# ap229997/hands

Measured on AMD Instinct MI355X. Metric: hands/sec, higher is better.
Workload: dtype f32; 1 GPU; hands_light ResNet-50 x3 + feature_conv + HMR + MANO, 224x224, bz=256 samples/GPU (512 hands, 768 trunk passes); per_gpu_batch=256, global_batch=256, parallelism=dp1, rccl_ranks=1, launched_by=direct, conv3x3_stride1=winograd_f4x4:stages1234

## Files before the change

hands_amd/csrc/conv_igemm.hip:

```cpp
#include <hip/hip_runtime.h>
#include <stdint.h>
#include "hands_hip.h"
#include "common.h"

namespace {

typedef unsigned int u32x4 __attribute__((ext_vector_type(4)));
typedef double f64x4 __attribute__((ext_vector_type(4)));

__device__ __forceinline__ float gelu_erf(float x) { return x * 0.5f * (1.0f + erff(x * 0.70710678118654752440f)); }

__device__ __forceinline__ float4 apply_act(float4 v, int act) {
  if (act == HANDS_ACT_RELU) {
    v = relu_f32(v);
  } else if (act == HANDS_ACT_GELU) {
    v.x = gelu_erf(v.x); v.y = gelu_erf(v.y); v.z = gelu_erf(v.z); v.w = gelu_erf(v.w);
  } else if (act == HANDS_ACT_LEAKY_RELU) {
    v.x = v.x > 0.f ? v.x : 0.01f * v.x; v.y = v.y > 0.f ? v.y : 0.01f * v.y;
    v.z = v.z > 0.f ? v.z : 0.01f * v.z; v.w = v.w > 0.f ? v.w : 0.01f * v.w;
  }
  return v;
}

__device__ __forceinline__ float f4elem(const float4& v, int t) {
  return t == 0 ? v.x : (t == 1 ? v.y : (t == 2 ? v.z : v.w));
}

constexpr int BK = 16;
constexpr int LDS_ROW = 16;
constexpr int LDS_ROW_B3 = 24;

typedef __bf16 bf16x8 __attribute__((ext_vector_type(8)));

__device__ __forceinline__ void split3(float x, uint32_t& u0, uint32_t& u1, uint32_t& u2) {
  u0 = __float_as_uint(x) & 0xffff0000u;
  const float r1 = x - __uint_as_float(u0);
  u1 = __float_as_uint(r1) & 0xffff0000u;
  const float r2 = r1 - __uint_as_float(u1);
  u2 = __float_as_uint(r2);
}

__device__ __forceinline__ void store_split4(float* dst, float4 v) {
  uint32_t a0, a1, a2, b0, b1, b2, c0, c1, c2, d0, d1, d2;
  split3(v.x, a0, a1, a2); split3(v.y, b0, b1, b2); split3(v.z, c0, c1, c2); split3(v.w, d0, d1, d2);
  *reinterpret_cast<uint2*>(dst) = make_uint2((a0 >> 16) | b0, (c0 >> 16) | d0);
  *reinterpret_cast<uint2*>(dst + 8) = make_uint2((a1 >> 16) | b1, (c1 >> 16) | d1);
  *reinterpret_cast<uint2*>(dst + 16) = make_uint2((a2 >> 16) | (b2 & 0xffff0000u), (c2 >> 16) | (d2 & 0xffff0000u));
}

struct ConvArgs {
  const float* __restrict__ in;
  const float* __restrict__ w;
  const float* __restrict__ bias;
  const float* res;
  float* out;
  int M, N, Kpad;
  int H, W, Cin, Ho, Wo, KH, KW, stride, pad;
  int in_ps, out_ps, res_ps;
  int relu;
  int nblk_m, nblk_n;
  const float* __restrict__ in2;
  int K0, H2, W2, stride2, in2_ps;
  int ksplit;
  float* partial;
  int part_ps;
  const float* pre_scale;
  const float* pre_shift;
  int* counters = nullptr;
  const float* fin_res = nullptr;
  int fin_act = 0;
};

__device__ __forceinline__ int xcd_remap(int bid, int nwg) {
  const int q = nwg >> 3, r = nwg & 7;
  const int xcd = bid & 7, idx = bid >> 3;
  const int base = (xcd < r) ? xcd * (q + 1) : r * (q + 1) + (xcd - r) * q;
  return base + idx;
}

typedef float f32x2 __attribute__((ext_vector_type(2)));

constexpr int EROW = 68;
constexpr int EPI_FLOATS = 4 * 32 * EROW;
template <int ACT, bool RES>
__device__ __forceinline__ void epilogue_full(const f32x16 (&acc)[2][2], float* sE, int lane, const float* bias_p,
                                              const char* res_u, int res_ps, char* out_u, int out_ps) {
  const int half = lane >> 5;
  float* wr = sE + (lane & 31) * EROW + half * 4;
  const float* rd = sE + (lane >> 4) * EROW + (lane & 15) * 4;
  const uint32_t o_off = (uint32_t)((lane >> 4) * out_ps + (lane & 15) * 4) * 4u;
  const uint32_t r_off = (uint32_t)((lane >> 4) * res_ps + (lane & 15) * 4) * 4u;
  const float4 bv4 = *reinterpret_cast<const float4*>(bias_p);
#ifndef HANDS_EPI_SCALAR_ADDS
  const f32x2 b01 = {bv4.x, bv4.y}, b23 = {bv4.z, bv4.w};
#endif
#pragma unroll
  for (int j = 0; j < 2; ++j) {
#pragma unroll
    for (int i = 0; i < 2; ++i)
#pragma unroll
      for (int q = 0; q < 4; ++q)
        *reinterpret_cast<float4*>(wr + i * 32 + q * 8) =
            make_float4(acc[i][j][q * 4 + 0], acc[i][j][q * 4 + 1], acc[i][j][q * 4 + 2], acc[i][j][q * 4 + 3]);
    float4 rv[RES ? 8 : 1];
    if constexpr (RES) {
#pragma unroll
      for (int r = 0; r < 8; ++r)
        rv[r] = *reinterpret_cast<const float4*>(res_u + (size_t)(j * 32 + 4 * r) * (size_t)res_ps * 4 + r_off);
    }
#pragma unroll
    for (int r = 0; r < 8; ++r) {
      const float4 t = *reinterpret_cast<const float4*>(rd + 4 * r * EROW);
#ifdef HANDS_EPI_SCALAR_ADDS
      float4 v = make_float4(t.x + bv4.x, t.y + bv4.y, t.z + bv4.z, t.w + bv4.w);
      if constexpr (RES) { v.x += rv[r].x; v.y += rv[r].y; v.z += rv[r].z; v.w += rv[r].w; }
      asm volatile("" : "+v"(v.x), "+v"(v.y), "+v"(v.z), "+v"(v.w));
#else
      f32x2 v01 = {t.x, t.y}, v23 = {t.z, t.w};
      v01 = v01 + b01;
      v23 = v23 + b23;
      if constexpr (RES) {
        const f32x2 r01 = {rv[r].x, rv[r].y}, r23 = {rv[r].z, rv[r].w};
        v01 = v01 + r01;
        v23 = v23 + r23;
      }
      float4 v = make_float4(v01.x, v01.y, v23.x, v23.y);
#endif
      if constexpr (ACT != HANDS_ACT_NONE) v = apply_act(v, ACT);
      *reinterpret_cast<float4*>(out_u + (size_t)(j * 32 + 4 * r) * (size_t)out_ps * 4 + o_off) = v;
      if (r & 1) __builtin_amdgcn_sched_barrier(0);
    }
  }
}

template <int BM, int BN, bool F64>
__device__ __forceinline__ void splitk_fused_tail(const ConvArgs& a, float* lds, int tile, int m0, int n0, int wave_u) {
  const int tid = wave_u * 64 + (int)__builtin_amdgcn_mbcnt_hi(~0u, __builtin_amdgcn_mbcnt_lo(~0u, 0u));
  volatile int& s_last = *reinterpret_cast<volatile int*>(lds);
  asm volatile("s_waitcnt vmcnt(0)" ::: "memory");
  __syncthreads();
  if (tid == 0) {
    __builtin_amdgcn_fence(__ATOMIC_RELEASE, "agent");
    asm volatile("s_waitcnt vmcnt(0)" ::: "memory");
    const int old = __hip_atomic_fetch_add(a.counters + tile, 1, __ATOMIC_RELAXED, __HIP_MEMORY_SCOPE_AGENT);
    const int last = old == a.ksplit - 1;
    if (last) __hip_atomic_store(a.counters + tile, 0, __ATOMIC_RELAXED, __HIP_MEMORY_SCOPE_AGENT);
    s_last = last;
  }
  __syncthreads();
  if (!s_last) return;
  __builtin_amdgcn_fence(__ATOMIC_ACQUIRE, "agent");
  const size_t slice = (size_t)a.M * a.part_ps;
  if constexpr (F64) {
    const double* part = reinterpret_cast<const double*>(a.partial);
    for (int idx = tid; idx < BM * BN; idx += 256) {
      const int m = m0 + idx / BN, n = n0 + idx % BN;
      if (m >= a.M || n >= a.N) continue;
      const double* p = part + (size_t)m * a.part_ps + n;
      double v = p[0];
      for (int sl = 1; sl < a.ksplit; ++sl) v += p[sl * slice];
      float f = (float)(v + (double)a.bias[n]);
      if (a.fin_res) f += a.fin_res[(size_t)m * a.res_ps + n];
      if (a.fin_act == HANDS_ACT_RELU) f = relu_f32(f);
      else if (a.fin_act == HANDS_ACT_GELU) f = gelu_erf(f);
      else if (a.fin_act == HANDS_ACT_LEAKY_RELU) f = f > 0.f ? f : 0.01f * f;
      a.out[(size_t)m * a.out_ps + n] = f;
    }
  } else {
    constexpr int C4 = BN / 4;
    for (int idx = tid; idx < BM * C4; idx += 256) {
      const int m = m0 + idx / C4, n = n0 + (idx % C4) * 4;
      if (m >= a.M || n >= a.N) continue;
      const float* p = a.partial + (size_t)m * a.part_ps + n;
      float4 v = *reinterpret_cast<const float4*>(p);
      for (int sl = 1; sl < a.ksplit; ++sl) {
        const float4 q = *reinterpret_cast<const float4*>(p + sl * slice);
        v.x += q.x; v.y += q.y; v.z += q.z; v.w += q.w;
      }
      const float4 b = *reinterpret_cast<const float4*>(a.bias + n);
      v.x += b.x; v.y += b.y; v.z += b.z; v.w += b.w;
      if (a.fin_res) {
        const float4 r = *reinterpret_cast<const float4*>(a.fin_res + (size_t)m * a.res_ps + n);
        v.x += r.x; v.y += r.y; v.z += r.z; v.w += r.w;
      }
      *reinterpret_cast<float4*>(a.out + (size_t)m * a.out_ps + n) = apply_act(v, a.fin_act);
    }
  }
}

constexpr int SK_SLOT_FLOATS = 4 * 64 * 64;

__device__ __forceinline__ void tile_coords(const ConvArgs& a, int tile, int& mt, int& nt) {
  constexpr int RASTER_GM = 8;
  if (a.nblk_n >= 8 && a.nblk_m >= RASTER_GM) {
    const int per = RASTER_GM * a.nblk_n;
    const int gidx = tile / per, idx = tile - gidx * per;
    const int gm = min(RASTER_GM, a.nblk_m - gidx * RASTER_GM);
    nt = idx / gm; mt = gidx * RASTER_GM + (idx - nt * gm);
  } else { mt = tile / a.nblk_n; nt = tile - mt * a.nblk_n; }
}

template <int WAVES_M, int WAVES_N, int MODE, int PREC = 0, bool PRE = false, int BLK = 0>
__device__ __forceinline__ void conv_tile(const ConvArgs& a, float* lds, int tile, int split, int kt0, int kt1,
                                          const float* acc_in, float* acc_out) {
  constexpr int ROW = PREC == 1 ? LDS_ROW_B3 : LDS_ROW;
  constexpr bool F64 = PREC == 2;
  constexpr bool STEM = MODE == 1;
  constexpr bool DUAL = MODE == 2;
  constexpr int BM = 64 * WAVES_M;
  constexpr int BN = 64 * WAVES_N;
  constexpr int A_ROWS = BM / 64;
  constexpr int W_ROWS = BN / 64;
  static_assert(WAVES_M * WAVES_N == 4, "4 waves per block");

  float* sX = lds;
  float* sW = lds + 2 * BM * ROW;

  const int tid = threadIdx.x;
  const int lane = tid & 63;
  const int wave = tid >> 6;
  const int wm = wave / WAVES_N;
  const int wn = wave % WAVES_N;

  int mt, nt;
  tile_coords(a, tile, mt, nt);
  const int m0 = mt * BM, n0 = nt * BN;

  const int srow = tid >> 2;
  const int chunk = tid & 3;
  const int swz_chunk = chunk ^ ((srow >> 2) & 3);
  int x_base[A_ROWS];
  int x_hi0[A_ROWS], x_wi0[A_ROWS];
  bool x_ok[A_ROWS];
  int x_base2[DUAL ? A_ROWS : 1];
  uint32_t x_mask[MODE == 0 ? A_ROWS : 1];
  int x_offb[MODE == 0 ? A_ROWS : 1];
  int x_b[A_ROWS];
  const int HoWo = a.Ho * a.Wo;
  const bool same_pixel = DUAL && a.K0 >= a.Kpad && a.stride == 1 && a.H == a.Ho && a.W == a.Wo;
#pragma unroll
  for (int i = 0; i < A_ROWS; ++i) {
    const int m = m0 + srow + 64 * i;
    x_ok[i] = m < a.M;
    const int mm = x_ok[i] ? m : 0;
    if (same_pixel) {
      x_b[i] = 0; x_hi0[i] = 0; x_wi0[i] = 0;
      x_base[i] = mm * a.in_ps;
      if constexpr (DUAL) x_base2[i] = 0;
      continue;
    }
    const int b = mm / HoWo;
    const int rem = mm - b * HoWo;
    const int ho = rem / a.Wo;
    const int wo = rem - ho * a.Wo;
    x_b[i] = b;
    x_hi0[i] = ho * a.stride - a.pad;
    x_wi0[i] = wo * a.stride - a.pad;
    x_base[i] = ((b * a.H + x_hi0[i]) * a.W + x_wi0[i]) * a.in_ps;
    if constexpr (DUAL) {
      x_base2[i] = ((b * a.H2 + ho * a.stride2) * a.W2 + wo * a.stride2) * a.in2_ps;
    }
  }
  __amdgpu_buffer_rsrc_t x_rsrc = __builtin_amdgcn_make_buffer_rsrc(const_cast<float*>(a.in), 0, (int)0x80000000u, 0x00020000);
  if constexpr (MODE == 0) {
    const int b_w = __builtin_amdgcn_readfirstlane(x_b[0]);
    x_rsrc = __builtin_amdgcn_make_buffer_rsrc(const_cast<float*>(a.in) + (size_t)b_w * a.H * a.W * a.in_ps, 0,
                                               (int)0x80000000u, 0x00020000);
#pragma unroll
    for (int i = 0; i < A_ROWS; ++i) {
      const int hb = max(0, -x_hi0[i]), he = min(a.KH, a.H - x_hi0[i]);
      const int wb = max(0, -x_wi0[i]), we = min(a.KW, a.W - x_wi0[i]);
      const uint32_t hm = he > hb ? ((1u << he) - 1u) & ~((1u << hb) - 1u) : 0u;
      const uint32_t wm = we > wb ? ((1u << we) - 1u) & ~((1u << wb) - 1u) : 0u;
      x_mask[i] = (x_ok[i] && hm != 0u && wm != 0u) ? (hm | (wm << 16)) : 0u;
      x_offb[i] = (((((x_b[i] - b_w) * a.H + x_hi0[i]) * a.W + x_wi0[i]) * a.in_ps) + chunk * 4) * 4;
    }
  }
  int x_off1[DUAL ? A_ROWS : 1], x_off2[DUAL ? A_ROWS : 1];
  __amdgpu_buffer_rsrc_t x_rsrc2 = x_rsrc;
  if constexpr (DUAL) {
    const int base1 = __builtin_amdgcn_readfirstlane(x_base[0]);
    const int base2 = __builtin_amdgcn_readfirstlane(x_base2[0]);
    x_rsrc = __builtin_amdgcn_make_buffer_rsrc(const_cast<float*>(a.in) + base1, 0, (int)0x80000000u, 0x00020000);
    x_rsrc2 = __builtin_amdgcn_make_buffer_rsrc(const_cast<float*>(a.in2) + base2, 0, (int)0x80000000u, 0x00020000);
#pragma unroll
    for (int i = 0; i < A_ROWS; ++i) {
      x_off1[i] = x_ok[i] ? (x_base[i] - base1 + chunk * 4) * 4 : chunk * 16;
      x_off2[i] = x_ok[i] ? (x_base2[i] - base2 + chunk * 4) * 4 : chunk * 16;
    }
  }
  const __amdgpu_buffer_rsrc_t w_rsrc =
      __builtin_amdgcn_make_buffer_rsrc(const_cast<float*>(a.w) + (size_t)n0 * a.Kpad, 0, (int)0x80000000u, 0x00020000);
  int w_offb[W_ROWS];
#pragma unroll
  for (int i = 0; i < W_ROWS; ++i) w_offb[i] = ((srow + 64 * i) * a.Kpad + chunk * 4) * 4;

  float4 xr[A_ROWS], wr[W_ROWS];
  static_assert(!PRE || (MODE == 2 && PREC != 1), "the input affine + LeakyReLU exists for exact-fp32 pointwise layers");
  float4 psr = make_float4(1.f, 1.f, 1.f, 1.f), pbr = make_float4(0.f, 0.f, 0.f, 0.f);
  int kh = 0, kw = 0, c0 = 0, woff = 0;
  const int ntaps = a.KH * a.KW;
  const int cw = (a.Cin & 31) == 0 ? 2 * BK : BK;

#define LOAD_TILES(KT)                                                                              \
  do {                                                                                              \
    if constexpr (STEM) {                                                                           \
                                          \
      const int tap = (KT) * 4 + chunk;                                                             \
      const int tkh = tap / a.KW;                                                                   \
      const int tkw = tap - tkh * a.KW;                                                             \
      const int toff = (tkh * a.W + tkw) * a.in_ps;                                                 \
      _Pragma("unroll") for (int i = 0; i < A_ROWS; ++i) {                                          \
        const bool ok = x_ok[i] && tap < ntaps && (unsigned)(x_hi0[i] + tkh) < (unsigned)a.H &&     \
                        (unsigned)(x_wi0[i] + tkw) < (unsigned)a.W;                                 \
        xr[i] = ok ? *reinterpret_cast<const float4*>(a.in + (x_base[i] + toff))                    \
                   : make_float4(0.f, 0.f, 0.f, 0.f);                                               \
      }                                                                                             \
    } else if constexpr (DUAL) {                                                                    \
       \
       \
       \
      const bool second = (KT) * BK >= a.K0;                                                        \
      const int soff = ((KT) * BK - (second ? a.K0 : 0)) * 4;                                       \
      _Pragma("unroll") for (int i = 0; i < A_ROWS; ++i) {                                          \
        const u32x4 ld = second ? __builtin_amdgcn_raw_buffer_load_b128(x_rsrc2, x_off2[i], soff, 0) \
                                : __builtin_amdgcn_raw_buffer_load_b128(x_rsrc, x_off1[i], soff, 0);  \
        xr[i] = make_float4(__uint_as_float(ld.x), __uint_as_float(ld.y), __uint_as_float(ld.z), __uint_as_float(ld.w)); \
      }                                                                                             \
    } else {                                                                                        \
       \
       \
       \
      const bool kvalid = c0 < a.Cin;              \
      const uint32_t sel = kvalid ? ((1u << kh) | (0x10000u << kw)) : 0x80000000u;   \
      const int toffb = ((kh * a.W + kw) * a.in_ps + c0) * 4;                                       \
      _Pragma("unroll") for (int i = 0; i < A_ROWS; ++i) {                                          \
        const bool ok = (x_mask[i] & sel) == sel;                                                   \
        const u32x4 ld = __builtin_amdgcn_raw_buffer_load_b128(x_rsrc, ok ? x_offb[i] + toffb : (int)0x80000000u, 0, 0); \
        xr[i] = make_float4(__uint_as_float(ld.x), __uint_as_float(ld.y), __uint_as_float(ld.z), __uint_as_float(ld.w)); \
      }                                                                                             \
      woff = kvalid ? (kh * a.KW + kw) * a.Cin + c0 : (KT) * BK;                                    \
      c0 += BK;                                                                                     \
      if ((c0 & (cw - 1)) == 0) {              \
        c0 -= cw;                                                                                   \
        if (++kw == a.KW) { kw = 0; if (++kh == a.KH) { kh = 0; c0 += cw; } }                       \
      }                                                                                             \
    }                                                                                               \
    if constexpr (MODE != 0) woff = (KT) * BK;                                                      \
    if constexpr (PRE) {                                                                            \
      psr = *reinterpret_cast<const float4*>(a.pre_scale + (KT) * BK + chunk * 4);                  \
      pbr = *reinterpret_cast<const float4*>(a.pre_shift + (KT) * BK + chunk * 4);                  \
    }                                                                                               \
    _Pragma("unroll") for (int i = 0; i < W_ROWS; ++i) {                                            \
      const u32x4 ld = __builtin_amdgcn_raw_buffer_load_b128(w_rsrc, w_offb[i], woff * 4, 0);        \
      wr[i] = make_float4(__uint_as_float(ld.x), __uint_as_float(ld.y), __uint_as_float(ld.z), __uint_as_float(ld.w)); \
    }                                                                                               \
  } while (0)

#define STORE_TILES(BUF)                                                                            \
  do {                                                                                              \
    if constexpr (PRE) {                                                                            \
      _Pragma("unroll") for (int i = 0; i < A_ROWS; ++i) {                                          \
        float4 v = make_float4(xr[i].x * psr.x + pbr.x, xr[i].y * psr.y + pbr.y, xr[i].z * psr.z + pbr.z, xr[i].w * psr.w + pbr.w); \
        v.x = v.x > 0.f ? v.x : 0.01f * v.x; v.y = v.y > 0.f ? v.y : 0.01f * v.y;                   \
        v.z = v.z > 0.f ? v.z : 0.01f * v.z; v.w = v.w > 0.f ? v.w : 0.01f * v.w;                   \
        xr[i] = v;                                                                                  \
      }                                                                                             \
    }                                                                                               \
    if constexpr (PREC != 1) {                                                                      \
      float* dx = sX + (BUF) * BM * ROW + srow * ROW + swz_chunk * 4;                               \
      float* dw = sW + (BUF) * BN * ROW + srow * ROW + swz_chunk * 4;                               \
      _Pragma("unroll") for (int i = 0; i < A_ROWS; ++i)                                            \
        *reinterpret_cast<float4*>(dx + 64 * i * ROW) = xr[i];                                      \
      _Pragma("unroll") for (int i = 0; i < W_ROWS; ++i)                                            \
        *reinterpret_cast<float4*>(dw + 64 * i * ROW) = wr[i];                                      \
    } else {                                                                                        \
      float* dx = sX + (BUF) * BM * ROW + srow * ROW + chunk * 2;                                   \
      float* dw = sW + (BUF) * BN * ROW + srow * ROW + chunk * 2;                                   \
      _Pragma("unroll") for (int i = 0; i < A_ROWS; ++i) store_split4(dx + 64 * i * ROW, xr[i]);    \
      _Pragma("unroll") for (int i = 0; i < W_ROWS; ++i) store_split4(dw + 64 * i * ROW, wr[i]);    \
    }                                                                                               \
  } while (0)

  f64x4 accd[F64 ? 4 : 1][F64 ? 4 : 1];
  if constexpr (F64) {
#pragma unroll
    for (int i = 0; i < 4; ++i)
#pragma unroll
      for (int j = 0; j < 4; ++j) accd[i][j] = f64x4{0.0, 0.0, 0.0, 0.0};
  }
  f32x16 acc[2][2];
  if (acc_in != nullptr) {
    const float4* src = reinterpret_cast<const float4*>(acc_in) + (wave * 16) * 64 + lane;
#pragma unroll
    for (int i = 0; i < 2; ++i)
#pragma unroll
      for (int j = 0; j < 2; ++j)
#pragma unroll
        for (int q = 0; q < 4; ++q) {
          const float4 v = src[((i * 2 + j) * 4 + q) * 64];
          acc[i][j][q * 4 + 0] = v.x; acc[i][j][q * 4 + 1] = v.y; acc[i][j][q * 4 + 2] = v.z; acc[i][j][q * 4 + 3] = v.w;
        }
  } else {
#pragma unroll
    for (int i = 0; i < 2; ++i)
#pragma unroll
      for (int j = 0; j < 2; ++j)
#pragma unroll
        for (int r = 0; r < 16; ++r) acc[i][j][r] = 0.f;
  }

  if constexpr (MODE == 0) {
    if (kt0 > 0) {
      const int spt = cw / BK;
      const int ch0 = kt0 / (ntaps * spt);
      const int r0 = kt0 - ch0 * ntaps * spt;
      const int tap0 = r0 / spt;
      c0 = ch0 * cw + (r0 - tap0 * spt) * BK;
      kh = tap0 / a.KW;
      kw = tap0 - kh * a.KW;
    }
  }
#ifdef HANDS_PRO_PRIO
  __builtin_amdgcn_s_setprio(HANDS_PRO_PRIO);
#endif
  LOAD_TILES(kt0);
  STORE_TILES(0);
  __syncthreads();
#ifdef HANDS_PRO_PRIO
  __builtin_amdgcn_s_setprio(0);
#endif

  const int frag = PREC == 1 ? (lane & 31) * ROW + (lane >> 5) * 4
                   : F64     ? (lane & 15) * ROW + (((lane >> 4) ^ ((lane >> 2) & 3)) * 4)
                             : (lane & 31) * ROW + (((lane >> 5) ^ ((lane >> 2) & 3)) * 4);
  const float* fw = sW + (wn * 64) * ROW + frag;
  const float* fx = sX + (wm * 64) * ROW + frag;
  const float* fw1 = sW + (wn * 64) * ROW + (frag ^ 8);
  const float* fx1 = sX + (wm * 64) * ROW + (frag ^ 8);

#define COMPUTE_STEP(BUF)                                                                           \
  do {                                                                                              \
    if constexpr (F64) {                                                                            \
      float4 wf[4], xf[4];                 \
      _Pragma("unroll") for (int i = 0; i < 4; ++i) {                                               \
        wf[i] = *reinterpret_cast<const float4*>(fw + (BUF) * BN * ROW + i * 16 * ROW);             \
        xf[i] = *reinterpret_cast<const float4*>(fx + (BUF) * BM * ROW + i * 16 * ROW);             \
      }                                                                                             \
      _Pragma("unroll") for (int t = 0; t < 4; ++t) {                                               \
        double wd[4], xd[4];                                                                        \
        _Pragma("unroll") for (int i = 0; i < 4; ++i) {                                             \
          wd[i] = (double)f4elem(wf[i], t);                                                         \
          xd[i] = (double)f4elem(xf[i], t);                                                         \
        }                                                                                           \
        _Pragma("unroll") for (int i = 0; i < 4; ++i) {                                             \
          _Pragma("unroll") for (int j = 0; j < 4; ++j) {                                           \
            accd[i][j] = __builtin_amdgcn_mfma_f64_16x16x4f64(wd[i], xd[j], accd[i][j], 0, 0, 0);   \
          }                                                                                         \
        }                                                                                           \
      }                                                                                             \
    } else if constexpr (PREC == 0) {                                                               \
      float4 wf[2][2], xf[2][2];                                            \
      _Pragma("unroll") for (int kk = 0; kk < 2; ++kk) {                                            \
        _Pragma("unroll") for (int i = 0; i < 2; ++i) {                                             \
          wf[i][kk] = *reinterpret_cast<const float4*>((kk ? fw1 : fw) + (BUF) * BN * ROW + i * 32 * ROW); \
          xf[i][kk] = *reinterpret_cast<const float4*>((kk ? fx1 : fx) + (BUF) * BM * ROW + i * 32 * ROW); \
        }                                                                                           \
      }                                                                                             \
      _Pragma("unroll") for (int kk = 0; kk < 2; ++kk) {                                            \
        _Pragma("unroll") for (int t = 0; t < 4; ++t) {                                             \
          _Pragma("unroll") for (int i = 0; i < 2; ++i) {                                           \
            _Pragma("unroll") for (int j = 0; j < 2; ++j) {                                         \
              acc[i][j] = __builtin_amdgcn_mfma_f32_32x32x2f32(f4elem(wf[i][kk], t), f4elem(xf[j][kk], t), \
                                                               acc[i][j], 0, 0, 0);                  \
            }                                                                                       \
          }                                                                                         \
        }                                                                                           \
      }                                                                                             \
    } else {                                                                                        \
        \
      bf16x8 wf[2][3], xf[2][3];                                         \
      _Pragma("unroll") for (int p = 0; p < 3; ++p) {                                               \
        _Pragma("unroll") for (int i = 0; i < 2; ++i) {                                             \
          wf[i][p] = *reinterpret_cast<const bf16x8*>(fw + (BUF) * BN * ROW + i * 32 * ROW + p * 8); \
          xf[i][p] = *reinterpret_cast<const bf16x8*>(fx + (BUF) * BM * ROW + i * 32 * ROW + p * 8); \
        }                                                                                           \
      }                                                                                             \
                             \
      _Pragma("unroll") for (int q = 0; q < 6; ++q) {                                               \
        constexpr int PA[6] = {2, 1, 0, 1, 0, 0};                                                   \
        constexpr int PB[6] = {0, 1, 2, 0, 1, 0};                                                   \
        _Pragma("unroll") for (int i = 0; i < 2; ++i) {                                             \
          _Pragma("unroll") for (int j = 0; j < 2; ++j) {                                           \
            acc[i][j] = __builtin_amdgcn_mfma_f32_32x32x16_bf16(wf[i][PA[q]], xf[j][PB[q]], acc[i][j], 0, 0, 0); \
          }                                                                                         \
        }                                                                                           \
      }                                                                                             \
    }                                                                                               \
  } while (0)

  static_assert(BLK == 0 || ((BLK & (BLK - 1)) == 0 && PREC == 0), "block length: a power of two k-steps, exact fp32 only");
  static_assert(!F64 || (WAVES_M == 2 && WAVES_N == 2), "fp64 accumulation: the 128 x 128 tile only");
  f32x16 tot[BLK ? 2 : 1][BLK ? 2 : 1];
  if constexpr (BLK > 0) {
#pragma unroll
    for (int i = 0; i < 2; ++i)
#pragma unroll
      for (int j = 0; j < 2; ++j)
#pragma unroll
        for (int r = 0; r < 16; ++r) tot[i][j][r] = 0.f;
  }
  for (int kt = kt0; kt + 1 < kt1; ++kt) {
    const int buf = (kt - kt0) & 1;
    LOAD_TILES(kt + 1);
    COMPUTE_STEP(buf);
    if constexpr (BLK > 0) {
      if (((kt - kt0 + 1) & (BLK - 1)) == 0) {
#pragma unroll
        for (int i = 0; i < 2; ++i)
#pragma unroll
          for (int j = 0; j < 2; ++j)
#pragma unroll
            for (int r = 0; r < 16; ++r) { tot[i][j][r] += acc[i][j][r]; acc[i][j][r] = 0.f; }
      }
    }
    STORE_TILES(buf ^ 1);
    __syncthreads();
  }
  COMPUTE_STEP((kt1 - 1 - kt0) & 1);
#ifdef HANDS_EPI_PRIO
  __builtin_amdgcn_s_setprio(HANDS_EPI_PRIO);
#endif
  if constexpr (BLK > 0) {
#pragma unroll
    for (int i = 0; i < 2; ++i)
#pragma unroll
      for (int j = 0; j < 2; ++j)
#pragma unroll
        for (int r = 0; r < 16; ++r) acc[i][j][r] += tot[i][j][r];
  }
#undef COMPUTE_STEP

  __syncthreads();
  if (acc_out != nullptr) {
    float4* dst = reinterpret_cast<float4*>(acc_out) + (wave * 16) * 64 + lane;
#pragma unroll
    for (int i = 0; i < 2; ++i)
#pragma unroll
      for (int j = 0; j < 2; ++j)
#pragma unroll
        for (int q = 0; q < 4; ++q)
          dst[((i * 2 + j) * 4 + q) * 64] =
              make_float4(acc[i][j][q * 4 + 0], acc[i][j][q * 4 + 1], acc[i][j][q * 4 + 2], acc[i][j][q * 4 + 3]);
    return;
  }
  float* sE = lds + wave * (32 * EROW);
  const int half = lane >> 5;
  const int c4 = lane & 15;
  const int n_lane = n0 + wn * 64 + c4 * 4;
  const bool n_ok = n_lane < a.N;
  const bool part = a.ksplit > 1;
#ifdef HANDS_ABL_NO_EPI
  if (!part && m0 + BM <= a.M && n0 + BN <= a.N) {
    float sacc = 0.f;
#pragma unroll
    for (int i = 0; i < 2; ++i)
#pragma unroll
      for (int j = 0; j < 2; ++j) sacc += acc[i][j][0] + acc[i][j][7] + acc[i][j][15];
    if (sacc == 123456.789f) a.out[(size_t)m0 * a.out_ps + n0 + lane] = sacc;
    return;
  }
#endif
  if (!F64 && !part && m0 + BM <= a.M && n0 + BN <= a.N) {
    const int wave_u = __builtin_amdgcn_readfirstlane(wave);
    const int mw = m0 + (wave_u / WAVES_N) * 64, nw = n0 + (wave_u % WAVES_N) * 64;
    char* ou = reinterpret_cast<char*>(a.out) + ((size_t)mw * a.out_ps + nw) * 4;
    const char* ru = reinterpret_cast<const char*>(a.res) + ((size_t)mw * a.res_ps + nw) * 4;
    const float* bp = a.bias + n_lane;
#define HANDS_EPI(ACT)                                                                            \
    if (a.res != nullptr) epilogue_full<ACT, true>(acc, sE, lane, bp, ru, a.res_ps, ou, a.out_ps); \
    else                  epilogue_full<ACT, false>(acc, sE, lane, bp, ru, a.res_ps, ou, a.out_ps)
    if (a.relu == HANDS_ACT_RELU) { HANDS_EPI(HANDS_ACT_RELU); }
    else if (a.relu == HANDS_ACT_NONE) { HANDS_EPI(HANDS_ACT_NONE); }
    else if (a.relu == HANDS_ACT_LEAKY_RELU) { HANDS_EPI(HANDS_ACT_LEAKY_RELU); }
    else { HANDS_EPI(HANDS_ACT_GELU); }
#undef HANDS_EPI
    return;
  }
  const float4 bv = (part || F64) ? make_float4(0.f, 0.f, 0.f, 0.f) : *reinterpret_cast<const float4*>(a.bias + n_lane);
  double bd[F64 ? 4 : 1][F64 ? 4 : 1];
  if constexpr (F64) {
#pragma unroll
    for (int i = 0; i < 4; ++i)
#pragma unroll
      for (int r = 0; r < 4; ++r) {
        const int ch = n0 + wn * 64 + 16 * i + (lane >> 4) + 4 * r;
        bd[i][r] = (!part && ch < a.N) ? (double)a.bias[ch] : 0.0;
      }
    if (part) {
      double* pd = reinterpret_cast<double*>(a.partial) + (size_t)split * a.M * a.part_ps;
#pragma unroll
      for (int i = 0; i < 4; ++i)
#pragma unroll
        for (int jb = 0; jb < 4; ++jb)
#pragma unroll
          for (int r = 0; r < 4; ++r) {
            const int ch = n0 + wn * 64 + 16 * i + (lane >> 4) + 4 * r;
            const int m = m0 + wm * 64 + 16 * jb + (lane & 15);
            if (m < a.M && ch < a.N) pd[(size_t)m * a.part_ps + ch] = accd[i][jb][r];
          }
      return;
    }
  }
  const bool has_res = !part && a.res != nullptr;
  const int act = part ? HANDS_ACT_NONE : a.relu;
  float* const obase = part ? a.partial + (size_t)split * a.M * a.part_ps : a.out;
  const int ops = part ? a.part_ps : a.out_ps;
#pragma unroll
  for (int j = 0; j < 2; ++j) {
    if constexpr (F64) {
#pragma unroll
      for (int i = 0; i < 4; ++i)
#pragma unroll
        for (int jj = 0; jj < 2; ++jj)
#pragma unroll
          for (int r = 0; r < 4; ++r)
            sE[(jj * 16 + (lane & 15)) * EROW + 16 * i + (lane >> 4) + 4 * r] = (float)(accd[i][2 * j + jj][r] + bd[i][r]);
    } else {
#pragma unroll
    for (int i = 0; i < 2; ++i)
#pragma unroll
      for (int q = 0; q < 4; ++q)
        *reinterpret_cast<float4*>(sE + (lane & 31) * EROW + i * 32 + q * 8 + half * 4) =
            make_float4(acc[i][j][q * 4 + 0], acc[i][j][q * 4 + 1], acc[i][j][q * 4 + 2], acc[i][j][q * 4 + 3]);
    }
    const int mbase = m0 + wm * 64 + j * 32 + (lane >> 4);
    float4 rv[8];
#pragma unroll
    for (int r = 0; r < 8; ++r) {
      const int m = mbase + 4 * r;
      const int mc = m < a.M ? m : a.M - 1;
      rv[r] = has_res ? *reinterpret_cast<const float4*>(a.res + (size_t)mc * a.res_ps + (n_ok ? n_lane : 0))
                      : make_float4(0.f, 0.f, 0.f, 0.f);
    }
#pragma unroll
    for (int r = 0; r < 8; ++r) {
      const int m = mbase + 4 * r;
      const float4 t = *reinterpret_cast<const float4*>(sE + ((lane >> 4) + 4 * r) * EROW + c4 * 4);
      float4 v;
      v.x = t.x + bv.x + rv[r].x;
      v.y = t.y + bv.y + rv[r].y;
      v.z = t.z + bv.z + rv[r].z;
      v.w = t.w + bv.w + rv[r].w;
      v = apply_act(v, act);
      if (m < a.M && n_ok) *reinterpret_cast<float4*>(obase + (size_t)m * ops + n_lane) = v;
    }
  }
#undef LOAD_TILES
#undef STORE_TILES
}

template <int WAVES_M, int WAVES_N, int MODE, int PREC = 0, bool PRE = false, int BLK = 0>
__global__ void __launch_bounds__(256, 2) conv_igemm_f32_kernel(ConvArgs a) {
  constexpr int RING = 2 * (64 * WAVES_M + 64 * WAVES_N) * (PREC == 1 ? LDS_ROW_B3 : LDS_ROW);
  __shared__ __attribute__((aligned(16))) float lds[RING > EPI_FLOATS ? RING : EPI_FLOATS];
  const int ntiles = a.nblk_m * a.nblk_n;
  const int split = a.ksplit > 1 ? blockIdx.x / ntiles : 0;
  const int tile = xcd_remap(a.ksplit > 1 ? blockIdx.x - split * ntiles : blockIdx.x, ntiles);
  const int nk_all = a.Kpad / BK;
  const int kt0 = a.ksplit > 1 ? (int)((long long)split * nk_all / a.ksplit) : 0;
  const int kt1 = a.ksplit > 1 ? (int)((long long)(split + 1) * nk_all / a.ksplit) : nk_all;
  const int wave_u = __builtin_amdgcn_readfirstlane((int)(threadIdx.x >> 6));
  conv_tile<WAVES_M, WAVES_N, MODE, PREC, PRE, BLK>(a, lds, tile, split, kt0, kt1, nullptr, nullptr);
  if (a.ksplit > 1 && a.counters != nullptr) {
    int mt, nt;
    tile_coords(a, tile, mt, nt);
    splitk_fused_tail<64 * WAVES_M, 64 * WAVES_N, PREC == 2>(a, lds, tile, mt * 64 * WAVES_M, nt * 64 * WAVES_N, wave_u);
  }
}

constexpr int GROUP_MAX = 8;
struct GroupArgs {
  ConvArgs a[GROUP_MAX];
  int start[GROUP_MAX + 1];
  int n;
};

template <int WAVES_M, int WAVES_N, int MODE, bool PRE, int BLK>
__global__ void __launch_bounds__(256, 2) conv_igemm_group_f32_kernel(GroupArgs g) {
  constexpr int RING = 2 * (64 * WAVES_M + 64 * WAVES_N) * LDS_ROW;
  __shared__ __attribute__((aligned(16))) float lds[RING > EPI_FLOATS ? RING : EPI_FLOATS];
  int p = 0;
#pragma unroll
  for (int i = 1; i < GROUP_MAX; ++i)
    if (i < g.n && (int)blockIdx.x >= g.start[i]) p = i;
  const ConvArgs& a = g.a[p];
  const int ntiles = a.nblk_m * a.nblk_n;
  const int local = (int)blockIdx.x - g.start[p];
  if ((local >> 3) >= (ntiles >> 3) + ((local & 7) < (ntiles & 7) ? 1 : 0)) return;
  conv_tile<WAVES_M, WAVES_N, MODE, 0, PRE, BLK>(a, lds, xcd_remap(local, ntiles), 0, 0, a.Kpad / BK, nullptr, nullptr);
}

struct SkArgs {
  float* slots;
  int* flags;
  int epoch;
};

template <int WAVES_M, int WAVES_N, int MODE>
__global__ void __launch_bounds__(256, 2) conv_igemm_sk_f32_kernel(ConvArgs a, SkArgs sk) {
  constexpr int RING = 2 * (64 * WAVES_M + 64 * WAVES_N) * LDS_ROW;
  __shared__ __attribute__((aligned(16))) float lds[RING > EPI_FLOATS ? RING : EPI_FLOATS];
  __shared__ int s_ready;
  const int G = gridDim.x;
  const int g = xcd_remap(blockIdx.x, G);
  const int ntiles = a.nblk_m * a.nblk_n;
  const int nk = a.Kpad / BK;
  const long long total = (long long)ntiles * nk;
  const long long u0 = total * g / G, u1 = total * (g + 1) / G;
  const int ta = (int)(u0 / nk), ka = (int)(u0 - (long long)ta * nk);
  const int tb = (int)(u1 / nk), kb = (int)(u1 - (long long)tb * nk);

  const bool inside = ta == tb;
  const int first_full = ka > 0 ? ta + 1 : ta;
  const int nfull = inside ? 0 : tb - first_full;
  const int head = (!inside && kb > 0) ? 1 : 0;
  const int nseg = inside ? 1 : head + nfull + (ka > 0 ? 1 : 0);
  for (int sgi = 0; sgi < nseg; ++sgi) {
    int tile, k0 = 0, k1 = nk;
    const float* ain = nullptr;
    float* aout = nullptr;
    if (sgi < head) {
      tile = tb; k1 = kb;
      aout = sk.slots + (size_t)g * SK_SLOT_FLOATS;
    } else if (sgi - head < nfull) {
      tile = first_full + (sgi - head);
    } else if (inside && ka == 0) {
      tile = ta; k1 = kb;
      aout = sk.slots + (size_t)g * SK_SLOT_FLOATS;
    } else {
      if (threadIdx.x == 0) {
        int ok = 0;
        for (int spin = 0; spin < 4096 && !ok; ++spin) {
          ok = __hip_atomic_load(sk.flags + (g - 1), __ATOMIC_RELAXED, __HIP_MEMORY_SCOPE_AGENT) == sk.epoch;
          if (!ok) __builtin_amdgcn_s_sleep(8);
        }
        if (ok) __builtin_amdgcn_fence(__ATOMIC_ACQUIRE, "agent");
        s_ready = ok;
      }
      __syncthreads();
      tile = ta;
      if (s_ready != 0) { k0 = ka; ain = sk.slots + (size_t)(g - 1) * SK_SLOT_FLOATS; }
      if (inside) { k1 = kb; aout = sk.slots + (size_t)g * SK_SLOT_FLOATS; }
    }
    __syncthreads();
    conv_tile<WAVES_M, WAVES_N, MODE>(a, lds, tile, 0, k0, k1, ain, aout);
    if (aout != nullptr) {
      asm volatile("s_waitcnt vmcnt(0)" ::: "memory");
      __syncthreads();
      if (threadIdx.x == 0) {
        __builtin_amdgcn_fence(__ATOMIC_RELEASE, "agent");
        asm volatile("s_waitcnt vmcnt(0)" ::: "memory");
        if (sk.epoch > 0) __hip_atomic_store(sk.flags + g, sk.epoch, __ATOMIC_RELAXED, __HIP_MEMORY_SCOPE_AGENT);
      }
    }
  }
}

template <int WAVES_M, int WAVES_N, int MODE, int PREC = 0, bool PRE = false, int BLK = 0>
int launch(ConvArgs& a, hipStream_t stream) {
  constexpr int BM = 64 * WAVES_M, BN = 64 * WAVES_N;
  a.nblk_m = (a.M + BM - 1) / BM;
  a.nblk_n = (a.N + BN - 1) / BN;
  const long long nwg = (long long)a.nblk_m * a.nblk_n * (a.ksplit > 1 ? a.ksplit : 1);
  if (nwg <= 0 || nwg > 0x7fffffffLL) return HANDS_EINVAL;
  hipLaunchKernelGGL((conv_igemm_f32_kernel<WAVES_M, WAVES_N, MODE, PREC, PRE, BLK>), dim3((unsigned)nwg), dim3(256), 0,
                     stream, a);
  return (int)hipGetLastError();
}

template <int MODE, bool PRE = false>
int launch_fp32(const hands_conv_desc* d, ConvArgs& a, hipStream_t s) {
  const bool narrow = d->Cout <= 64;
  if (d->act & HANDS_ACC_F64) return launch<2, 2, MODE, 2, PRE>(a, s);
  if (d->act & HANDS_SUM_BLOCK128) return narrow ? launch<4, 1, MODE, 0, PRE, 8>(a, s) : launch<2, 2, MODE, 0, PRE, 8>(a, s);
  if (d->act & HANDS_SUM_BLOCK64) return narrow ? launch<4, 1, MODE, 0, PRE, 4>(a, s) : launch<2, 2, MODE, 0, PRE, 4>(a, s);
  return narrow ? launch<4, 1, MODE, 0, PRE>(a, s) : launch<2, 2, MODE, 0, PRE>(a, s);
}

constexpr int SK_MAX_G = 1024;

int device_cus() {
  static int cus = 0;
  if (cus == 0) {
    int dev = 0, n = 0;
    if (hipGetDevice(&dev) == hipSuccess &&
        hipDeviceGetAttribute(&n, hipDeviceAttributeMultiprocessorCount, dev) == hipSuccess && n > 0)
      cus = n;
    else
      cus = 256;
  }
  return cus;
}

template <int WAVES_M, int WAVES_N, int MODE>
int sk_blocks_per_cu() {
  static int occ = 0;
  if (occ == 0) {
    int n = 0;
    if (hipOccupancyMaxActiveBlocksPerMultiprocessor(&n, conv_igemm_sk_f32_kernel<WAVES_M, WAVES_N, MODE>, 256, 0) != hipSuccess || n < 1)
      n = 1;
    occ = n > 4 ? 4 : n;
  }
  return occ;
}

int streamk_grid(long long ntiles, int nk, int cus, int max_per_cu) {
  if (ntiles > cus + cus / 8 && ntiles < 2LL * cus && nk >= 128 && max_per_cu >= 2) {
    return 2 * cus;
  }
  if (nk < 16 || ntiles < 2LL * cus || ntiles > 8LL * cus) return 0;
  const double per_cu = (double)ntiles / cus;
  const long long rounds = (ntiles + cus - 1) / cus;
  if (per_cu / (double)rounds > 0.95) return 0;
  long long j = ntiles / cus;
  if (j > max_per_cu) j = max_per_cu;
  long long G = j * cus;
  if (G > SK_MAX_G) G = SK_MAX_G / cus * cus;
  return G >= cus ? (int)G : 0;
}

template <int WAVES_M, int WAVES_N, int MODE>
int launch_streamk(ConvArgs& a, hipStream_t stream, void* workspace, long long workspace_bytes, int epoch) {
  constexpr int BM = 64 * WAVES_M, BN = 64 * WAVES_N;
  a.nblk_m = (a.M + BM - 1) / BM;
  a.nblk_n = (a.N + BN - 1) / BN;
  const long long ntiles = (long long)a.nblk_m * a.nblk_n;
  const int G = (workspace && epoch != 0 && a.ksplit <= 1)
                    ? streamk_grid(ntiles, a.Kpad / BK, device_cus(), sk_blocks_per_cu<WAVES_M, WAVES_N, MODE>()) : 0;
  const long long need = (long long)G * SK_SLOT_FLOATS * 4 + (long long)SK_MAX_G * 4;
  if (G == 0 || workspace_bytes < need) return launch<WAVES_M, WAVES_N, MODE>(a, stream);
  SkArgs sk;
  sk.flags = reinterpret_cast<int*>(workspace);
  sk.slots = reinterpret_cast<float*>(reinterpret_cast<char*>(workspace) + SK_MAX_G * 4);
  sk.epoch = epoch;
  hipLaunchKernelGGL((conv_igemm_sk_f32_kernel<WAVES_M, WAVES_N, MODE>), dim3((unsigned)G), dim3(256), 0, stream, a, sk);
  return (int)hipGetLastError();
}

__global__ void splitk_reduce_kernel(const float* __restrict__ partial, int S, int M, int N4, int part_ps,
                                     const float* __restrict__ bias, const float* res, int res_ps, float* out, int out_ps,
                                     int act) {
  const long long total = (long long)M * N4;
  for (long long i = blockIdx.x * (long long)blockDim.x + threadIdx.x; i < total; i += (long long)gridDim.x * blockDim.x) {
    const int n = (int)(i % N4) * 4;
    const long long m = i / N4;
    float4 v = *reinterpret_cast<const float4*>(partial + m * part_ps + n);
    for (int s = 1; s < S; ++s) {
      const float4 p = *reinterpret_cast<const float4*>(partial + ((long long)s * M + m) * part_ps + n);
      v.x += p.x; v.y += p.y; v.z += p.z; v.w += p.w;
    }
    const float4 b = *reinterpret_cast<const float4*>(bias + n);
    v.x += b.x; v.y += b.y; v.z += b.z; v.w += b.w;
    if (res) {
      const float4 r = *reinterpret_cast<const float4*>(res + m * res_ps + n);
      v.x += r.x; v.y += r.y; v.z += r.z; v.w += r.w;
    }
    *reinterpret_cast<float4*>(out + m * out_ps + n) = apply_act(v, act);
  }
}

__global__ void splitk_reduce_f64_kernel(const double* __restrict__ partial, int S, int M, int N, int part_ps,
                                         const float* __restrict__ bias, const float* res, int res_ps, float* out, int out_ps,
                                         int act) {
  const long long total = (long long)M * N;
  for (long long i = blockIdx.x * (long long)blockDim.x + threadIdx.x; i < total; i += (long long)gridDim.x * blockDim.x) {
    const int n = (int)(i % N);
    const long long m = i / N;
    double v = partial[m * part_ps + n];
    for (int s = 1; s < S; ++s) v += partial[((long long)s * M + m) * part_ps + n];
    float f = (float)(v + (double)bias[n]);
    if (res) f += res[m * res_ps + n];
    if (act == HANDS_ACT_RELU) f = relu_f32(f);
    else if (act == HANDS_ACT_GELU) f = gelu_erf(f);
    else if (act == HANDS_ACT_LEAKY_RELU) f = f > 0.f ? f : 0.01f * f;
    out[m * out_ps + n] = f;
  }
}

int splitk_factor(const hands_conv_desc* d) {
  if (d->KH != 1 || d->KW != 1 || d->H != 1 || d->W != 1 || d->stride != 1 || d->pad != 0 || d->Cin == 4) return 1;
  const long long M = d->B;
  if (M > 2048 || d->Kpad < 512) return 1;
  int s = d->Kpad / 256;
  return s > 8 ? 8 : s;
}

bool conv_geometry_ok(const hands_conv_desc* d) {
  if (d->B <= 0 || d->H <= 0 || d->W <= 0 || d->Ho <= 0 || d->Wo <= 0 || d->KH <= 0 || d->KW <= 0 || d->stride <= 0 ||
      d->pad < 0)
    return false;
  if ((d->act & HANDS_ACT_MASK) > HANDS_ACT_LEAKY_RELU || (d->act & ~(HANDS_ACT_MASK | HANDS_MATH_BF16X3 | HANDS_SUM_BLOCK128 | HANDS_SUM_BLOCK64 | HANDS_ACC_F64))) return false;
  if ((d->act & HANDS_ACC_F64) && ((d->act & (HANDS_MATH_BF16X3 | HANDS_SUM_BLOCK128 | HANDS_SUM_BLOCK64)) || d->Cin == 4)) return false;
  if ((d->act & HANDS_SUM_BLOCK128) && (d->act & (HANDS_SUM_BLOCK64 | HANDS_MATH_BF16X3))) return false;
  if ((d->act & HANDS_SUM_BLOCK64) && (d->act & HANDS_MATH_BF16X3)) return false;
  if (d->Cin % 4 || d->Cout % 4 || d->Kpad % BK || d->Kpad < d->KH * d->KW * d->Cin) return false;
  if (d->Cin != 4 && d->Cin % 16) return false;
  if (d->in_pix_stride < d->Cin || d->out_pix_stride < d->Cout) return false;
  if (d->in_pix_stride % 4 || d->out_pix_stride % 4) return false;
  if (d->H + 2 * d->pad < d->KH || d->W + 2 * d->pad < d->KW) return false;
  if (d->Ho > (d->H + 2 * d->pad - d->KH) / d->stride + 1 || d->Wo > (d->W + 2 * d->pad - d->KW) / d->stride + 1) return false;
  if ((long long)d->B * d->H * d->W * d->in_pix_stride >= (1LL << 31)) return false;
  if (d->Cin != 4) {
    const long long imgs = 256 / ((long long)d->Ho * d->Wo) + 2;
    if (imgs * d->H * d->W * d->in_pix_stride * 4 >= (1LL << 31)) return false;
    if (256LL * d->Kpad * 4 >= (1LL << 31)) return false;
    if (!(d->KH == 1 && d->KW == 1 && d->pad == 0) && (d->KH > 15 || d->KW > 15)) return false;
  }
  return true;
}

bool residual_ok(const hands_conv_desc* d, const float* residual) {
  return residual == nullptr || (d->res_pix_stride >= 0 && d->res_pix_stride % 4 == 0);
}

bool pointwise_route_ok(const hands_conv_desc* d) {
  return d->KH == 1 && d->KW == 1 && d->pad == 0 && d->Cin != 4 && d->Kpad == d->Cin &&
         (long long)(d->Ho - 1) * d->stride < d->H && (long long)(d->Wo - 1) * d->stride < d->W;
}

void fill_plain_args(const hands_conv_desc* d, const float* in, const float* w_packed, const float* bias, const float* residual,
                     float* out, const float* pre_scale, const float* pre_shift, ConvArgs& a) {
  a.in = in; a.w = w_packed; a.bias = bias; a.res = residual; a.out = out;
  a.M = d->B * d->Ho * d->Wo; a.N = d->Cout; a.Kpad = d->Kpad;
  a.H = d->H; a.W = d->W; a.Cin = d->Cin; a.Ho = d->Ho; a.Wo = d->Wo;
  a.KH = d->KH; a.KW = d->KW; a.stride = d->stride; a.pad = d->pad;
  a.in_ps = d->in_pix_stride; a.out_ps = d->out_pix_stride; a.res_ps = d->res_pix_stride;
// ... 220 lines not shown
```

Baseline: 12050 hands/s.

## Prefetch residual rows before last MFMA step and hoist epilogue loads

Issues the first four residual-tile loads before the final compute step so their latency overlaps the last MFMA block, and stages the first accumulator half to LDS before the epilogue dispatch. For ReLU/none activations it also loads both halves' residual rows up front. The aim is to hide the residual-read latency in the fused epilogue, at the cost of more live VGPRs, which may lower occupancy or cause spills.

```diff
diff --git a/hands_amd/csrc/conv_igemm.hip b/hands_amd/csrc/conv_igemm.hip
--- a/hands_amd/csrc/conv_igemm.hip
+++ b/hands_amd/csrc/conv_igemm.hip
@@ -82,45 +82,58 @@
 
 constexpr int EROW = 68;
 constexpr int EPI_FLOATS = 4 * 32 * EROW;
-template <int ACT, bool RES>
+constexpr int EPI_PRE = 4;
+
+__device__ __forceinline__ void epi_stage(const f32x16 (&acc)[2][2], int j, float* sE, int lane) {
+  float* wr = sE + (lane & 31) * EROW + (lane >> 5) * 4;
+#pragma unroll
+  for (int i = 0; i < 2; ++i)
+#pragma unroll
+    for (int q = 0; q < 4; ++q)
+      *reinterpret_cast<float4*>(wr + i * 32 + q * 8) =
+          make_float4(acc[i][j][q * 4 + 0], acc[i][j][q * 4 + 1], acc[i][j][q * 4 + 2], acc[i][j][q * 4 + 3]);
+}
+
+__device__ __forceinline__ uint32_t epi_lane_off(int lane, int ps) { return (uint32_t)((lane >> 4) * ps + (lane & 15) * 4) * 4u; }
+__device__ __forceinline__ float4 epi_res_row(const char* res_u, int res_ps, uint32_t r_off, int row) {
+  return *reinterpret_cast<const float4*>(res_u + (size_t)row * (size_t)res_ps * 4 + r_off);
+}
+
+template <int ACT, bool RES, int NPRE>
 __device__ __forceinline__ void epilogue_full(const f32x16 (&acc)[2][2], float* sE, int lane, const float* bias_p,
-                                              const char* res_u, int res_ps, char* out_u, int out_ps) {
-  const int half = lane >> 5;
-  float* wr = sE + (lane & 31) * EROW + half * 4;
+                                              const char* res_u, int res_ps, char* out_u, int out_ps, const float4* pre) {
   const float* rd = sE + (lane >> 4) * EROW + (lane & 15) * 4;
-  const uint32_t o_off = (uint32_t)((lane >> 4) * out_ps + (lane & 15) * 4) * 4u;
-  const uint32_t r_off = (uint32_t)((lane >> 4) * res_ps + (lane & 15) * 4) * 4u;
+  const uint32_t o_off = epi_lane_off(lane, out_ps);
+  const uint32_t r_off = epi_lane_off(lane, res_ps);
   const float4 bv4 = *reinterpret_cast<const float4*>(bias_p);
 #ifndef HANDS_EPI_SCALAR_ADDS
   const f32x2 b01 = {bv4.x, bv4.y}, b23 = {bv4.z, bv4.w};
 #endif
+  constexpr bool BOTH = RES && (ACT == HANDS_ACT_NONE || ACT == HANDS_ACT_RELU);
+  float4 rv[RES ? 2 : 1][RES ? 8 : 1];
 #pragma unroll
   for (int j = 0; j < 2; ++j) {
-#pragma unroll
-    for (int i = 0; i < 2; ++i)
-#pragma unroll
-      for (int q = 0; q < 4; ++q)
-        *reinterpret_cast<float4*>(wr + i * 32 + q * 8) =
-            make_float4(acc[i][j][q * 4 + 0], acc[i][j][q * 4 + 1], acc[i][j][q * 4 + 2], acc[i][j][q * 4 + 3]);
-    float4 rv[RES ? 8 : 1];
+    if (j == 1) epi_stage(acc, 1, sE, lane);
     if constexpr (RES) {
 #pragma unroll
-      for (int r = 0; r < 8; ++r)
-        rv[r] = *reinterpret_cast<const float4*>(res_u + (size_t)(j * 32 + 4 * r) * (size_t)res_ps * 4 + r_off);
+      for (int r = 0; r < 8; ++r) {
+        if (j == 0) rv[0][r] = r < NPRE ? pre[r] : epi_res_row(res_u, res_ps, r_off, 4 * r);
+        if (j == (BOTH ? 0 : 1)) rv[1][r] = epi_res_row(res_u, res_ps, r_off, 32 + 4 * r);
+      }
     }
 #pragma unroll
     for (int r = 0; r < 8; ++r) {
       const float4 t = *reinterpret_cast<const float4*>(rd + 4 * r * EROW);
 #ifdef HANDS_EPI_SCALAR_ADDS
       float4 v = make_float4(t.x + bv4.x, t.y + bv4.y, t.z + bv4.z, t.w + bv4.w);
-      if constexpr (RES) { v.x += rv[r].x; v.y += rv[r].y; v.z += rv[r].z; v.w += rv[r].w; }
+      if constexpr (RES) { v.x += rv[j][r].x; v.y += rv[j][r].y; v.z += rv[j][r].z; v.w += rv[j][r].w; }
       asm volatile("" : "+v"(v.x), "+v"(v.y), "+v"(v.z), "+v"(v.w));
 #else
       f32x2 v01 = {t.x, t.y}, v23 = {t.z, t.w};
       v01 = v01 + b01;
       v23 = v23 + b23;
       if constexpr (RES) {
-        const f32x2 r01 = {rv[r].x, rv[r].y}, r23 = {rv[r].z, rv[r].w};
+        const f32x2 r01 = {rv[j][r].x, rv[j][r].y}, r23 = {rv[j][r].z, rv[j][r].w};
         v01 = v01 + r01;
         v23 = v23 + r23;
       }
@@ -527,6 +540,19 @@
     STORE_TILES(buf ^ 1);
     __syncthreads();
   }
+  constexpr int NPRE = (PREC == 0 && BLK == 0) ? EPI_PRE : 0;
+  float4 rpre[NPRE ? NPRE : 1];
+  if constexpr (NPRE > 0) {
+    if (a.res != nullptr && (a.relu == HANDS_ACT_NONE || a.relu == HANDS_ACT_RELU) && acc_out == nullptr && a.ksplit <= 1 &&
+        m0 + BM <= a.M && n0 + BN <= a.N) {
+      const int wave_u = __builtin_amdgcn_readfirstlane(wave);
+      const int mw = m0 + (wave_u / WAVES_N) * 64, nw = n0 + (wave_u % WAVES_N) * 64;
+      const char* ru = reinterpret_cast<const char*>(a.res) + ((size_t)mw * a.res_ps + nw) * 4;
+      const uint32_t r_off = epi_lane_off(lane, a.res_ps);
+#pragma unroll
+      for (int r = 0; r < NPRE; ++r) rpre[r] = epi_res_row(ru, a.res_ps, r_off, 4 * r);
+    }
+  }
   COMPUTE_STEP((kt1 - 1 - kt0) & 1);
 #ifdef HANDS_EPI_PRIO
   __builtin_amdgcn_s_setprio(HANDS_EPI_PRIO);
@@ -571,19 +597,20 @@
     return;
   }
 #endif
+  if constexpr (!F64) epi_stage(acc, 0, sE, lane);
   if (!F64 && !part && m0 + BM <= a.M && n0 + BN <= a.N) {
     const int wave_u = __builtin_amdgcn_readfirstlane(wave);
     const int mw = m0 + (wave_u / WAVES_N) * 64, nw = n0 + (wave_u % WAVES_N) * 64;
+    const char* ru = reinterpret_cast<const char*>(a.res) + ((size_t)mw * a.res_ps + nw) * 4;
     char* ou = reinterpret_cast<char*>(a.out) + ((size_t)mw * a.out_ps + nw) * 4;
-    const char* ru = reinterpret_cast<const char*>(a.res) + ((size_t)mw * a.res_ps + nw) * 4;
     const float* bp = a.bias + n_lane;
-#define HANDS_EPI(ACT)                                                                            \
-    if (a.res != nullptr) epilogue_full<ACT, true>(acc, sE, lane, bp, ru, a.res_ps, ou, a.out_ps); \
-    else                  epilogue_full<ACT, false>(acc, sE, lane, bp, ru, a.res_ps, ou, a.out_ps)
-    if (a.relu == HANDS_ACT_RELU) { HANDS_EPI(HANDS_ACT_RELU); }
-    else if (a.relu == HANDS_ACT_NONE) { HANDS_EPI(HANDS_ACT_NONE); }
-    else if (a.relu == HANDS_ACT_LEAKY_RELU) { HANDS_EPI(HANDS_ACT_LEAKY_RELU); }
-    else { HANDS_EPI(HANDS_ACT_GELU); }
+#define HANDS_EPI(ACT, NP)                                                                                  \
+    if (a.res != nullptr) epilogue_full<ACT, true, NP>(acc, sE, lane, bp, ru, a.res_ps, ou, a.out_ps, rpre); \
+    else                  epilogue_full<ACT, false, 0>(acc, sE, lane, bp, ru, a.res_ps, ou, a.out_ps, rpre)
+    if (a.relu == HANDS_ACT_RELU) { HANDS_EPI(HANDS_ACT_RELU, NPRE); }
+    else if (a.relu == HANDS_ACT_NONE) { HANDS_EPI(HANDS_ACT_NONE, NPRE); }
+    else if (a.relu == HANDS_ACT_LEAKY_RELU) { HANDS_EPI(HANDS_ACT_LEAKY_RELU, 0); }
+    else { HANDS_EPI(HANDS_ACT_GELU, 0); }
 #undef HANDS_EPI
     return;
   }
@@ -626,13 +653,8 @@
 #pragma unroll
           for (int r = 0; r < 4; ++r)
             sE[(jj * 16 + (lane & 15)) * EROW + 16 * i + (lane >> 4) + 4 * r] = (float)(accd[i][2 * j + jj][r] + bd[i][r]);
-    } else {
-#pragma unroll
-    for (int i = 0; i < 2; ++i)
-#pragma unroll
-      for (int q = 0; q < 4; ++q)
-        *reinterpret_cast<float4*>(sE + (lane & 31) * EROW + i * 32 + q * 8 + half * 4) =
-            make_float4(acc[i][j][q * 4 + 0], acc[i][j][q * 4 + 1], acc[i][j][q * 4 + 2], acc[i][j][q * 4 + 3]);
+    } else if (j == 1) {
+      epi_stage(acc, 1, sE, lane);
     }
     const int mbase = m0 + wm * 64 + j * 32 + (lane >> 4);
     float4 rv[8];
```

New measurement: 12030 hands/s. About the same (-0.2%).
